# rpng/cpi

Measured on AMD Instinct MI355X. Metric: preintegration windows/sec (50-sample windows), higher is better.
Workload: dtype f64; 1 GPU; v1_mean: 10000 windows x 50 samples per GPU per step, CPI model 1, mean-only (BASELINE.json configs[1]); pool_batches=12, library_build=3afb5072f8491ca2, launch_mode=1923 timed steps replayed as ONE HIP graph (one kernel node per step), parallelism=1 GPU

## Files before the change

### cpi_amd/_lib.py

```python
import ctypes as C
import os

_HERE = os.path.dirname(os.path.abspath(__file__))
LIB_PATH = os.environ.get("CPI_AMD_LIB") or os.path.join(_HERE, "libcpi_amd.so")

CPI_OK, CPI_ERR_INVALID, CPI_ERR_HIP, CPI_ERR_NO_DEVICE, CPI_ERR_RCCL = 0, 1, 2, 3, 4
ABI_VERSION = 3
OUT_FIELDS = [("DT", 1), ("alpha", 3), ("beta", 3), ("q", 4), ("J_q", 9), ("J_a", 9), ("J_b", 9),
              ("H_a", 9), ("H_b", 9), ("O_a", 9), ("O_b", 9), ("P", 225), ("P_sym", 120)]
TRI_DOUBLES = 120


class CpiParams(C.Structure):
    _fields_ = [("sigma_w", C.c_double), ("sigma_wb", C.c_double), ("sigma_a", C.c_double),
                ("sigma_ab", C.c_double), ("grav", C.c_double * 3), ("model", C.c_int32),
                ("imu_avg", C.c_int32), ("state_transition_jacobians", C.c_int32),
                ("lanes_per_window", C.c_int32)]


class CpiOutputs(C.Structure):
    _fields_ = [(name, C.c_void_p) for name, _ in OUT_FIELDS]


class CpiLmParams(C.Structure):
# ... 27 lines not shown
    from . import build as _build
    hipcc_missing = None if (os.path.exists(_build.HIPCC) or shutil.which(_build.HIPCC)) else "no %s on this machine" % _build.HIPCC
    if LIB_PATH == _build.LIB and not hipcc_missing:
        if _build.stale():
            _build.build()
        elif _embedded_build_id(LIB_PATH) != _build.source_id():
            _build.build(force=True)
    if not os.path.exists(LIB_PATH):
        raise ImportError("cpi_amd: %s is missing and could not be built (%r); no CPU fallback exists" % (LIB_PATH, hipcc_missing))
    lib = C.CDLL(LIB_PATH)
    vp, i32, i64, dp = C.c_void_p, C.c_int32, C.c_int64, C.c_void_p
    lib.cpi_abi_version.restype = C.c_int
    if lib.cpi_abi_version() != ABI_VERSION:
        raise ImportError("cpi_amd: %s has ABI version %d, this binding expects %d (stale build?)" % (LIB_PATH, lib.cpi_abi_version(), ABI_VERSION))
    missing = [n for n in ("cpi_preintegrate_stream", "cpi_assemble_tiles", "cpi_tile_windows", "cpi_outputs_bind_slab", "cpi_preintegrate_tiled_batch_host",
                          "cpi_preintegrate_stream_host", "cpi_sqrt_information_packed_batch", "cpi_factor_eval_whitened_tri_batch",
                          "cpi_factor_hessian_tri_batch", "cpi_group_gather_chunk", "cpi_shard_chunk_bounds")
               if not hasattr(lib, n)]
    if missing:
        raise ImportError("cpi_amd: %s lacks %s (an older build: run python -m cpi_amd.build --force)" % (LIB_PATH, ", ".join(missing)))
    lib.cpi_build_id.restype = C.c_char_p
    if LIB_PATH == _build.LIB:
        have, want = (lib.cpi_build_id() or b"").decode(), _build.source_id()
        if have != want:
            msg = "cpi_amd: %s was built from other sources than this tree holds (build id %s, sources %s)%s" % (
                LIB_PATH, have, want, "; hipcc is not available here (%r)" % (hipcc_missing,) if hipcc_missing else "")
            if os.environ.get("CPI_AMD_ALLOW_STALE") != "1":
                raise ImportError(msg + " -- run python -m cpi_amd.build --force, or set CPI_AMD_ALLOW_STALE=1 to load it anyway")
            import warnings
            warnings.warn(msg + " (CPI_AMD_ALLOW_STALE=1: loaded anyway)")
    lib.cpi_group_create.argtypes = [C.c_int, C.POINTER(C.c_int), C.POINTER(vp)]
    lib.cpi_group_destroy.argtypes = [vp]
    lib.cpi_group_destroy.restype = None
    lib.cpi_group_size.argtypes = [vp]
    lib.cpi_group_ctx.argtypes = [vp, C.c_int]
    lib.cpi_group_ctx.restype = vp
    lib.cpi_group_last_error.argtypes = [vp]
    lib.cpi_group_last_error.restype = C.c_char_p
    lib.cpi_shard_bounds.argtypes = [i64, C.c_int, C.c_int, C.POINTER(i64), C.POINTER(i64)]
    lib.cpi_shard_bounds.restype = None
    lib.cpi_group_gather.argtypes = [vp, C.c_int, i64, C.POINTER(CpiOutputs), C.POINTER(CpiOutputs)]
    lib.cpi_group_gather_chunk.argtypes = [vp, C.c_int, i64, C.c_int, C.c_int, C.POINTER(CpiOutputs), C.POINTER(CpiOutputs)]
    lib.cpi_shard_chunk_bounds.argtypes = [i64, C.c_int, C.c_int, C.c_int, C.c_int, C.POINTER(i64), C.POINTER(i64)]
    lib.cpi_shard_chunk_bounds.restype = None
    lib.cpi_group_synchronize.argtypes = [vp]
    lib.cpi_ctx_create.argtypes = [C.c_int, vp, C.POINTER(vp)]
    lib.cpi_ctx_destroy.argtypes = [vp]
    lib.cpi_ctx_destroy.restype = None
    lib.cpi_last_error.argtypes = [vp]
    lib.cpi_last_error.restype = C.c_char_p
    lib.cpi_ctx_synchronize.argtypes = [vp]
    lib.cpi_ctx_set_stream.argtypes = [vp, vp]
    lib.cpi_ctx_set_capture_overlap.argtypes = [vp, i32]
    lib.cpi_preintegrate_batch.argtypes = [vp, C.POINTER(CpiParams), i64, i32, dp, vp, vp, dp, dp, C.POINTER(CpiOutputs)]
    lib.cpi_preintegrate_tiled_batch.argtypes = [vp, C.POINTER(CpiParams), i64, i32, dp, vp, dp, dp, C.POINTER(CpiOutputs)]
    lib.cpi_tile_knots.argtypes = [vp, i64, i32, dp, dp]
    lib.cpi_stream_workspace_bytes.argtypes = [i64]
    lib.cpi_stream_workspace_bytes.restype = C.c_size_t
    lib.cpi_stream_counts.argtypes = [vp, i64]
    lib.cpi_stream_counts.restype = C.c_void_p
    lib.cpi_preintegrate_stream.argtypes = [vp, C.POINTER(CpiParams), i64, dp, i64, dp, i32, dp, dp, vp, C.POINTER(CpiOutputs)]
    lib.cpi_preintegrate_stream.restype = C.c_int
    lib.cpi_preintegrate_stream_host.argtypes = [vp, C.POINTER(CpiParams), i64, dp, i64, dp, i32, dp, dp, C.POINTER(CpiOutputs), vp]
    lib.cpi_streams_workspace_bytes.argtypes = [i64, i64]
    lib.cpi_streams_workspace_bytes.restype = C.c_size_t
    lib.cpi_preintegrate_streams.argtypes = [vp, C.POINTER(CpiParams), i64, i64, dp, vp, i64, dp, vp, i32, dp, dp, vp, C.POINTER(CpiOutputs)]
    lib.cpi_preintegrate_streams_host.argtypes = [vp, C.POINTER(CpiParams), i64, i64, dp, vp, i64, dp, vp, i32, dp, dp, C.POINTER(CpiOutputs), vp]
    lib.cpi_tile_windows.argtypes = [vp, i64, i32, dp, vp, vp, dp]
    lib.cpi_assemble_tiles.argtypes = [vp, i64, dp, i64, dp, i32, dp, vp]
    lib.cpi_preintegrate_tiled_batch_host.argtypes = [vp, C.POINTER(CpiParams), i64, i32, dp, vp, dp, dp, C.POINTER(CpiOutputs)]
    lib.cpi_outputs_slab_doubles.argtypes = [C.POINTER(CpiOutputs), i64]
    lib.cpi_outputs_slab_doubles.restype = C.c_size_t
    lib.cpi_outputs_bind_slab.argtypes = [C.POINTER(CpiOutputs), i64, dp, C.POINTER(CpiOutputs)]
    lib.cpi_group_last_gather_messages.argtypes = [vp]
    if hasattr(lib, "cpi_test_group_create_shared"):
        lib.cpi_test_group_create_shared.argtypes = [C.c_int, C.c_int, C.POINTER(vp)]
        lib.cpi_test_group_create_shared.restype = C.c_int
        lib.cpi_test_quat_ops.argtypes = [vp, i32, i64, dp, dp]
        lib.cpi_test_quat_ops.restype = C.c_int
    lib.cpi_factor_eval_batch.argtypes = [vp, i32, C.POINTER(C.c_double), i64, C.POINTER(CpiOutputs), dp, dp, dp, i64, vp, vp, dp, dp, dp]
    lib.cpi_factor_eval_packed_batch.argtypes = [vp, i32, C.POINTER(C.c_double), i64, C.POINTER(CpiOutputs), dp, dp, dp, i64, vp, vp, dp]
    lib.cpi_sqrt_information_batch.argtypes = [vp, i64, dp, dp]
    lib.cpi_sqrt_information_packed_batch.argtypes = [vp, i64, dp, dp]
    lib.cpi_factor_eval_whitened_tri_batch.argtypes = [vp, i32, C.POINTER(C.c_double), i64, C.POINTER(CpiOutputs), dp, dp, dp, i64, vp, vp, dp, dp, dp, dp]
    lib.cpi_factor_hessian_tri_batch.argtypes = [vp, i32, C.POINTER(C.c_double), i64, C.POINTER(CpiOutputs), dp, dp, dp, i64, vp, vp, dp, dp]
    lib.cpi_factor_eval_whitened_batch.argtypes = [vp, i32, C.POINTER(C.c_double), i64, C.POINTER(CpiOutputs), dp, dp, dp, i64, vp, vp, dp, dp, dp, dp]
    lib.cpi_factor_hessian_batch.argtypes = [vp, i32, C.POINTER(C.c_double), i64, C.POINTER(CpiOutputs), dp, dp, dp, i64, vp, vp, dp, dp]
    lib.cpi_predict_batch.argtypes = [vp, i32, C.POINTER(C.c_double), i64, C.POINTER(CpiOutputs), dp, i64, vp, dp]
    lib.cpi_preintegrate_batch_host.argtypes = [vp, C.POINTER(CpiParams), i64, i32, dp, vp, vp, i64, dp, dp, C.POINTER(CpiOutputs)]
    lib.cpi_carry_doubles.argtypes = [i32]
    lib.cpi_carry_doubles.restype = C.c_size_t
    lib.cpi_preintegrate_resume.argtypes = [vp, C.POINTER(CpiParams), i64, i32, dp, vp, vp, dp, dp, dp, dp, C.POINTER(CpiOutputs)]
    lib.cpi_preintegrate_resume_host.argtypes = [vp, C.POINTER(CpiParams), i64, i32, dp, vp, vp, i64, dp, dp, dp, dp, C.POINTER(CpiOutputs)]
    lib.cpi_preintegrate_running.argtypes = [vp, C.POINTER(CpiParams), i64, i32, dp, vp, vp, dp, dp, C.POINTER(CpiOutputs)]
    lib.cpi_preintegrate_running_host.argtypes = [vp, C.POINTER(CpiParams), i64, i32, dp, vp, vp, i64, dp, dp, C.POINTER(CpiOutputs)]
    lib.cpi_preintegrate_running_resume.argtypes = lib.cpi_preintegrate_resume.argtypes
    lib.cpi_preintegrate_running_resume_host.argtypes = lib.cpi_preintegrate_resume_host.argtypes
    lib.cpi_preintegrate_running_resume.restype = lib.cpi_preintegrate_running_resume_host.restype = C.c_int
    lib.cpi_query_batch.argtypes = [vp, C.POINTER(CpiParams), i64, i32, dp, vp, vp, dp, dp, C.POINTER(CpiOutputs), i64, vp, dp, C.POINTER(CpiOutputs)]
    lib.cpi_query_batch_host.argtypes = [vp, C.POINTER(CpiParams), i64, i32, dp, vp, vp, i64, dp, dp, i64, vp, dp, C.POINTER(CpiOutputs)]
    lib.cpi_query_batch.restype = lib.cpi_query_batch_host.restype = C.c_int
    lib.cpi_query_cov_batch.argtypes = lib.cpi_query_batch.argtypes
    lib.cpi_query_cov_batch_host.argtypes = lib.cpi_query_batch_host.argtypes
    lib.cpi_query_cov_batch.restype = lib.cpi_query_cov_batch_host.restype = C.c_int
    lib.cpi_query_stj_batch.argtypes = lib.cpi_query_cov_batch.argtypes
    lib.cpi_query_stj_batch_host.argtypes = lib.cpi_query_cov_batch_host.argtypes
# ... 77 lines not shown
```

### cpi_amd/csrc/cpi_abi.hip

```cpp
#include <hip/hip_runtime.h>
#include <rccl/rccl.h>
#include <dlfcn.h>
#include <stdlib.h>
#include <stdint.h>
#include <stdio.h>
#include <string.h>
#include <algorithm>
#include <cmath>
#include <mutex>
#include <string>
#include <vector>

#include "../../include/cpi_amd.h"
#ifdef CPI_TEST_HOOKS
#include "../../include/cpi_amd_test.h"
#endif
#include "cpi_args.hpp"
#include "cpi_capture_overlap.hpp"

using namespace cpi;

constexpr int kOutFields = 13;
static_assert(sizeof(cpi_outputs) == kOutFields * sizeof(double *), "cpi_outputs is a plain table of kOutFields pointers");
static const int OUT_N[kOutFields] = { 1, 3, 3, 4, 9, 9, 9, 9, 9, 9, 9, 225, CPI_TRI_DOUBLES };
static double **out_field(cpi_outputs *o, int k) {
    double **f[kOutFields] = { &o->DT, &o->alpha, &o->beta, &o->q, &o->J_q, &o->J_a, &o->J_b, &o->H_a, &o->H_b, &o->O_a, &o->O_b, &o->P, &o->P_sym };
    return f[k];
}
static double *out_field_c(const cpi_outputs *o, int k) { cpi_outputs t = *o; return *out_field(&t, k); }

struct HostPipe;
static void host_pipe_destroy(HostPipe *);
struct cpi_ctx {
    int device;
    hipStream_t stream;
    std::string err;
    hipStream_t side = nullptr;
    hipEvent_t ev_fork = nullptr, ev_join = nullptr;
    unsigned big_lds_set = 0;
    struct HostPipe *pipe = nullptr;
    int overlap_depth = 1;
    bool overlap_allowed = true;
    overlap::Window<hipGraphNode_t> window;
    std::vector<hipGraphNode_t> ov_found, ov_preds;
};
static thread_local std::string g_create_err;

static int fail(cpi_ctx *ctx, int code, const std::string &msg) {
    if (ctx) ctx->err = msg; else g_create_err = msg;
    return code;
}
struct DeviceGuard {
    int prev = -1;
    bool changed = false;
    hipError_t enter(int dev) {
        hipError_t e = hipGetDevice(&prev);
        if (e != hipSuccess) return e;
        if (prev == dev) return hipSuccess;
        e = hipSetDevice(dev);
        changed = (e == hipSuccess);
        return e;
    }
    ~DeviceGuard() { if (changed) (void)hipSetDevice(prev); }
};
#define CPI_HIP(ctx, call)                                                                      \
    do {                                                                                        \
        hipError_t e_ = (call);                                                                 \
        if (e_ != hipSuccess)                                                                   \
            return fail(ctx, CPI_ERR_HIP, std::string(#call) + ": " + hipGetErrorString(e_));   \
    } while (0)

extern "C" int cpi_abi_version(void) { return CPI_ABI_VERSION; }
#ifndef CPI_BUILD_ID
#define CPI_BUILD_ID "unknown"
#endif
static const char kBuildIdTagged[] = "cpi-build-id:" CPI_BUILD_ID;
extern "C" const char *cpi_build_id(void) { return kBuildIdTagged + 13; }

extern "C" int cpi_ctx_create(int device, void *stream, cpi_ctx **out) {
    if (!out) return fail(nullptr, CPI_ERR_INVALID, "cpi_ctx_create: out is NULL");
    *out = nullptr;
    int ndev = 0;
    hipError_t e = hipGetDeviceCount(&ndev);
    if (e != hipSuccess || ndev <= 0)
        return fail(nullptr, CPI_ERR_NO_DEVICE, "cpi_ctx_create: no HIP device available (this library has no CPU fallback)");
    if (device < 0) {
        e = hipGetDevice(&device);
        if (e != hipSuccess) return fail(nullptr, CPI_ERR_HIP, std::string("hipGetDevice: ") + hipGetErrorString(e));
    }
    if (device >= ndev) return fail(nullptr, CPI_ERR_INVALID, "cpi_ctx_create: device index out of range");
    cpi_ctx *c = new cpi_ctx();
    c->device = device;
    c->stream = (hipStream_t)stream;
    const overlap::Policy pol = overlap::policy_from_environment();
    c->overlap_allowed = pol.allowed;
    c->overlap_depth = pol.depth;
    *out = c;
    return CPI_OK;
}
extern "C" void cpi_ctx_destroy(cpi_ctx *ctx) {
    if (!ctx) return;
    if (ctx->side || ctx->pipe) {
        int prev = -1;
        (void)hipGetDevice(&prev);
        (void)hipSetDevice(ctx->device);
        if (ctx->side) {
            (void)hipStreamDestroy(ctx->side);
            (void)hipEventDestroy(ctx->ev_fork);
            (void)hipEventDestroy(ctx->ev_join);
        }
        if (ctx->pipe) host_pipe_destroy(ctx->pipe);
        if (prev >= 0) (void)hipSetDevice(prev);
    }
    delete ctx;
}
extern "C" int cpi_ctx_set_stream(cpi_ctx *ctx, void *stream) {
    if (!ctx) return fail(nullptr, CPI_ERR_INVALID, "ctx is NULL");
    if (ctx->stream != (hipStream_t)stream) ctx->window.close();
    ctx->stream = (hipStream_t)stream;
    return CPI_OK;
}
extern "C" int cpi_ctx_set_capture_overlap(cpi_ctx *ctx, int32_t depth) {
    if (!ctx) return fail(nullptr, CPI_ERR_INVALID, "ctx is NULL");
    ctx->overlap_depth = ctx->overlap_allowed ? overlap::clamp_depth(depth) : 1;
    ctx->window.close();
    return CPI_OK;
}
extern "C" const char *cpi_last_error(const cpi_ctx *ctx) { return ctx ? ctx->err.c_str() : g_create_err.c_str(); }
extern "C" int cpi_ctx_synchronize(cpi_ctx *ctx) {
    if (!ctx) return fail(nullptr, CPI_ERR_INVALID, "ctx is NULL");
    DeviceGuard guard_;
    CPI_HIP(ctx, guard_.enter(ctx->device));
    CPI_HIP(ctx, hipStreamSynchronize(ctx->stream));
    return CPI_OK;
}

static bool grid_ok(long long nb) { return nb > 0 && nb <= 0x7fffffffLL; }

#ifdef CPI_EXPERIMENTS
namespace expsw {
static launch::MeanDmaCfg mean_dma() {
    static launch::MeanDmaCfg c = [] {
        launch::MeanDmaCfg d = {0, 0, 0};
        const char *e = getenv("CPI_AMD_MEAN_DMA");
        if (e && strcmp(e, "off") != 0) { int k = 0, s = 0, al = 1; if (sscanf(e, "%d,%d,%d", &k, &s, &al) >= 2) d = {k, s, al}; }
        return d;
    }();
    return c;
}
static int env_int(const char *name, int dflt) { const char *e = getenv(name); return e ? atoi(e) : dflt; }
static int mean_blk() { static int v = [] { const char *e = getenv("CPI_AMD_MEAN_BLK"); return e ? (strcmp(e, "off") == 0 ? -1 : atoi(e)) : 0; }(); return v; }
static bool mean_line() { static int v = env_int("CPI_AMD_MEAN_LINE", 0); return v != 0; }
static int blk_mode() { static int v = env_int("CPI_AMD_BLK_MODE", 0); return v; }
static int probe_lds() { static int v = env_int("CPI_AMD_PROBE_LDS", 0); return v; }
static bool no_overlap() { static int v = env_int("CPI_AMD_NO_OVERLAP", 0); return v != 0; }
static bool no_fused_cut() { static int v = env_int("CPI_AMD_NO_FUSED_CUT", 0); return v != 0; }
static int factor_lanes() { static int v = env_int("CPI_AMD_FACTOR_LANES", 0); return (v == 16 || v == 8 || v == 4) ? v : 0; }
static int cost_lanes() { static int v = env_int("CPI_AMD_COST_LANES", 0); return (v == 16 || v == 8 || v == 4) ? v : 0; }
static int packed_lpf() { static int v = env_int("CPI_AMD_PACKED_LPF", 0); return (v == 2 || v == 3 || v == 4 || v == 6 || v == 8) ? v : 0; }
}
#endif

static int pick_lanes(const cpi_params *prm, int64_t W, int N, bool jac) {
    if (prm->model == CPI_MODEL_V2 && jac) return 1;
    const double t_int = (prm->model == CPI_MODEL_V2) ? 1.2 : 0.55, t_lvl = (prm->model == CPI_MODEL_V2) ? 1.3 : 0.3;
    int L = prm->lanes_per_window;
    if (L <= 0) {
        double best = 1e300;
        L = 1;
        const int *choices = nullptr;
        const int nc = launch::mean_lane_choices(&choices);
        for (int i = 0; i < nc; i++) {
            const int c = choices[i];
            if (c > 1 && 2 * c > N) break;
            const int64_t waves = (W + (64 / c) - 1) / (64 / c);
            if (c > 1 && waves > 1024) break;
            int levels = 0;
            while ((1 << levels) < c) levels++;
// ... 77 lines not shown
                         const double *lin, const double *q_k_lin) {
    if (!knots || !lin) return refuse(ctx, who, "knots/lin is NULL");
    CPI_TRY(check_qk(ctx, who, prm, q_k_lin));
    CPI_TRY(check_grid(ctx, who, "W", W, " (32-bit grid)"));
    CPI_TRY(check_N(ctx, who, N));
    return check_lanes(ctx, prm);
}
static int check_carry_overlap(cpi_ctx *ctx, const char *who, const cpi_params *prm, int64_t W, const double *carry_in, const double *carry_out) {
    const int64_t n = W * (int64_t)carry::doubles(prm->model);
    return (carry_in && carry_in < carry_out + n && carry_out < carry_in + n) ? refuse(ctx, who, "carry_in and carry_out overlap") : CPI_OK;
}
static int carry_header(const cpi_params *prm) {
    const bool stj = prm->model == CPI_MODEL_V2 && prm->state_transition_jacobians != 0;
    return 1 | (prm->imu_avg != 0 ? 8 : 0) | (stj ? 16 : 0) | (32 * prm->model);
}

static int side_fork(cpi_ctx *ctx) {
    if (!ctx->side) {
        CPI_HIP(ctx, hipStreamCreateWithFlags(&ctx->side, hipStreamNonBlocking));
        CPI_HIP(ctx, hipEventCreateWithFlags(&ctx->ev_fork, hipEventDisableTiming));
        CPI_HIP(ctx, hipEventCreateWithFlags(&ctx->ev_join, hipEventDisableTiming));
    }
    CPI_HIP(ctx, hipEventRecord(ctx->ev_fork, ctx->stream));
    CPI_HIP(ctx, hipStreamWaitEvent(ctx->side, ctx->ev_fork, 0));
    return CPI_OK;
}
static int side_join(cpi_ctx *ctx) {
    CPI_HIP(ctx, hipEventRecord(ctx->ev_join, ctx->side));
    CPI_HIP(ctx, hipStreamWaitEvent(ctx->stream, ctx->ev_join, 0));
    return CPI_OK;
}

struct StreamCut {
    long long K;
    const double *update;
    long long *first;
    int *count;
    double *tstart, *tend;
    const RunArgs *runs;
};
static int cut_launch(cpi_ctx *ctx, const StreamCut &sc, const double *stream, int64_t U, int32_t N) {
    if (sc.runs) launch::cut_runs(sc.K, stream, (long long)U, sc.update, *sc.runs, sc.first, sc.count, sc.tstart, sc.tend, ctx->stream);
    else launch::cut_windows(sc.K, stream, (long long)U, sc.update, (int)N, sc.first, sc.count, sc.tstart, sc.tend, ctx->stream);
    CPI_HIP(ctx, hipGetLastError());
    return CPI_OK;
}
static void overlap_give_up(cpi_ctx *ctx, bool restore) {
    (void)hipGetLastError();
    if (restore) {
        (void)hipStreamUpdateCaptureDependencies(ctx->stream, ctx->ov_found.empty() ? nullptr : ctx->ov_found.data(), ctx->ov_found.size(),
                                                 hipStreamAddCaptureDependencies);
        (void)hipGetLastError();
    }
    ctx->window.close();
}
static bool capture_overlap_begin(cpi_ctx *ctx, const overlap::Footprint &fp) {
    if (ctx->overlap_depth <= 1 || !ctx->stream) return false;
    hipStreamCaptureStatus status = hipStreamCaptureStatusNone;
    unsigned long long id = 0;
    const hipGraphNode_t *deps = nullptr;
    size_t ndeps = 0;
    if (hipStreamGetCaptureInfo_v2(ctx->stream, &status, &id, nullptr, &deps, &ndeps) != hipSuccess) { overlap_give_up(ctx, false); return false; }
    if (status != hipStreamCaptureStatusActive || (ndeps && !deps)) { ctx->window.close(); return false; }
    if (!overlap::capture_registry().sole(id, ctx)) { ctx->window.close(); return false; }
    ctx->ov_found.assign(deps, deps + ndeps);
    if (!ctx->window.continues(id, ctx->ov_found.data(), ndeps)) ctx->window.open_at(id, ctx->overlap_depth, ctx->ov_found.data(), ndeps);
    ctx->window.plan(fp, ctx->ov_preds);
    if (overlap::same_set(ctx->ov_preds, ctx->ov_found.data(), ndeps)) return true;
    if (hipStreamUpdateCaptureDependencies(ctx->stream, ctx->ov_preds.empty() ? nullptr : ctx->ov_preds.data(), ctx->ov_preds.size(),
                                           hipStreamSetCaptureDependencies) != hipSuccess) {
        overlap_give_up(ctx, true);
        return false;
    }
    return true;
}
static void capture_overlap_end(cpi_ctx *ctx, const overlap::Footprint &fp) {
    hipStreamCaptureStatus status = hipStreamCaptureStatusNone;
    unsigned long long id = 0;
    const hipGraphNode_t *deps = nullptr;
    size_t ndeps = 0;
    if (hipStreamGetCaptureInfo_v2(ctx->stream, &status, &id, nullptr, &deps, &ndeps) != hipSuccess ||
        status != hipStreamCaptureStatusActive || ndeps != 1 || !deps) { overlap_give_up(ctx, true); return; }
    const hipGraphNode_t node = deps[0];
    for (hipGraphNode_t p : ctx->ov_preds) if (p == node) { overlap_give_up(ctx, true); return; }
    ctx->window.commit(node, fp);
    const std::vector<hipGraphNode_t> &fr = ctx->window.frontier();
    if (fr.size() == 1) return;
    if (hipStreamUpdateCaptureDependencies(ctx->stream, const_cast<hipGraphNode_t *>(fr.data()), fr.size(), hipStreamSetCaptureDependencies) != hipSuccess)
        overlap_give_up(ctx, true);
}

static int preintegrate_impl(cpi_ctx *ctx, const char *who, const cpi_params *prm, int64_t W, int32_t N, const double *knots,
                             const int64_t *first, const int32_t *count, const StreamCut *sc, const double *lin,
                             const double *q_k_lin, const cpi_outputs *out) {
    if (!ctx) return fail(nullptr, CPI_ERR_INVALID, "ctx is NULL");
    if (!prm || !out) return refuse(ctx, who, "prm/out is NULL");
    if (!model_is_cpi(prm) && prm->model != CPI_MODEL_FORSTER) return refuse(ctx, who, "model must be 1, 2 or 3 (CPI_MODEL_FORSTER)");
    if (W < 0 || N < 0) return refuse(ctx, who, "negative size");
    if (W == 0) return CPI_OK;
    CPI_TRY(check_windows(ctx, who, prm, W, N, knots, lin, q_k_lin));

    const Request rq = request_of(out);
    const bool forster = prm->model == CPI_MODEL_FORSTER;
    const bool avg = prm->imu_avg != 0;
    const bool v2 = prm->model == CPI_MODEL_V2;
    const bool stj = v2 && prm->state_transition_jacobians != 0;
    const bool run_cov = !forster && (rq.cov || (stj && rq.jac));
    const bool mean_jac = !forster && rq.jac && !stj;
    const bool run_mean = !forster && (mean_jac || (rq.mean && !run_cov));
    bool fused_cut = sc && rq.any() && run_mean && !mean_jac && !run_cov && (sc->runs != nullptr || sc->K >= 4);
#ifdef CPI_EXPERIMENTS
    if (expsw::no_fused_cut()) fused_cut = false;
#endif

    bool overlap_ok = !sc && run_mean && !run_cov;
#ifdef CPI_EXPERIMENTS
    overlap_ok = overlap_ok && expsw::mean_blk() <= 0 && expsw::mean_dma().kc <= 0 && !expsw::mean_line();
#endif

    DeviceGuard guard_;
    CPI_HIP(ctx, guard_.enter(ctx->device));
    if (!overlap_ok) ctx->window.close();
    if (sc && !fused_cut) {
        CPI_TRY(cut_launch(ctx, *sc, knots, W, N));
        first = reinterpret_cast<const int64_t *>(sc->first); count = sc->count;
    }
    if (!rq.any()) return CPI_OK;
    PreArgs a = pre_args(prm, W, N, knots, first, count, lin, q_k_lin, out);
    if (sc) { a.K = sc->K; if (!fused_cut) { a.tstart = sc->tstart; a.tend = sc->tend; } }
    if (forster) {
        launch::forster(a, ctx->stream);
        CPI_HIP(ctx, hipGetLastError());
        return CPI_OK;
    }

    bool forked = run_cov && run_mean && mean_jac;
#ifdef CPI_EXPERIMENTS
    forked = forked && !expsw::no_overlap();
#endif
    if (forked) CPI_TRY(side_fork(ctx));
    const hipStream_t mean_stream = forked ? ctx->side : ctx->stream;
    if (run_cov) {
        PreArgs c = a;
        c.write_means = rq.mean ? 1 : 0;
        c.write_jac = (stj && rq.jac) ? 1 : 0;
        launch::cov(prm->model, avg, c, ctx->stream);
    }
    if (run_mean) {
        PreArgs m = a;
        m.write_means = (rq.mean && !run_cov) ? 1 : 0;
        m.write_jac = mean_jac ? 1 : 0;
        if (fused_cut) { m.update = sc->update; m.count_out = sc->count; m.first = nullptr; m.count = nullptr; }
        const int LL = pick_lanes(prm, W, N, mean_jac);
        long long done = 0;
#ifdef CPI_EXPERIMENTS
        const int bl = expsw::mean_blk();
        m.dbg = expsw::blk_mode();
        if (!sc && !mean_jac && !first && bl > 0 && (size_t)(64 / bl) * (size_t)(N + 1) * 56 <= 65536 && N >= 1) {
            if (launch::mean_blk(prm->model, bl, avg, m, ctx->stream)) done = W;
        }
        const launch::MeanDmaCfg dc = expsw::mean_dma();
        if (!sc && !done && !mean_jac && LL == 1 && !first && !count && dc.kc > 0 && N >= 2 * dc.kc)
            done = launch::mean_dma(prm->model, dc, avg, m, ctx->stream);
        if (!sc && !done && !mean_jac && LL == 1 && !first && !count && expsw::mean_line()) done = launch::mean_line(prm->model, avg, m, ctx->stream);
        if (done && done < W) m = shift_windows(m, done);
#endif
        if (done < W) {
            if (fused_cut && sc->runs) launch::mean_runs(prm->model, avg, LL, m, *sc->runs, mean_stream);
            else if (overlap_ok && ctx->overlap_depth > 1 && !overlap::launch_is_latency_bound((W + (64 / LL) - 1) / (64 / LL))) {
                ctx->window.close();
                launch::mean(prm->model, mean_jac, avg, LL, m, mean_stream);
            } else if (overlap_ok && ctx->overlap_depth > 1) {
                const void *outs[kOutFields];
                for (int k = 0; k < kOutFields; k++) outs[k] = out_field_c(out, k);
                const overlap::Footprint fp = overlap::make_footprint(W, N, knots, first, count, lin, q_k_lin, outs, OUT_N, kOutFields);
                const bool in_window = capture_overlap_begin(ctx, fp);
                launch::mean(prm->model, mean_jac, avg, LL, m, mean_stream);
                const hipError_t launched = hipGetLastError();
                if (in_window) capture_overlap_end(ctx, fp);
                CPI_HIP(ctx, launched);
            } else launch::mean(prm->model, mean_jac, avg, LL, m, mean_stream);
        }
    }
    if (forked) CPI_TRY(side_join(ctx));
    CPI_HIP(ctx, hipGetLastError());
    return CPI_OK;
}
extern "C" int cpi_preintegrate_batch(cpi_ctx *ctx, const cpi_params *prm, int64_t W, int32_t N,
                                      const double *knots, const int64_t *first, const int32_t *count,
                                      const double *lin, const double *q_k_lin, const cpi_outputs *out) {
    return preintegrate_impl(ctx, "cpi_preintegrate_batch", prm, W, N, knots, first, count, nullptr, lin, q_k_lin, out);
}

extern "C" size_t cpi_carry_doubles(int32_t model) { return (model == CPI_MODEL_V1 || model == CPI_MODEL_V2) ? (size_t)carry::doubles(model) : 0; }
extern "C" int cpi_preintegrate_resume(cpi_ctx *ctx, const cpi_params *prm, int64_t W, int32_t N,
                                       const double *knots, const int64_t *first, const int32_t *count,
                                       const double *lin, const double *q_k_lin, const double *carry_in, double *carry_out,
                                       const cpi_outputs *out) {
    static const char who[] = "cpi_preintegrate_resume";
    if (!ctx) return fail(nullptr, CPI_ERR_INVALID, "ctx is NULL");
    if (!prm || !out) return refuse(ctx, who, "prm/out is NULL");
    if (!model_is_cpi(prm)) return refuse_forster(ctx, who, NOT_RESUMABLE);
    if (!carry_out) return refuse(ctx, who, "carry_out is NULL");
    if (W < 0 || N < 0) return refuse(ctx, who, "negative size");
    CPI_TRY(check_carry_overlap(ctx, who, prm, W, carry_in, carry_out));
    if (W == 0) return CPI_OK;
    CPI_TRY(check_windows(ctx, who, prm, W, N, knots, lin, q_k_lin));

    const Request rq = request_of(out);
    const bool avg = prm->imu_avg != 0;
    const bool stj = prm->model == CPI_MODEL_V2 && prm->state_transition_jacobians != 0;
    const bool run_cov = rq.cov || (stj && rq.jac);
    const bool mean_jac = rq.jac && !stj;
    const bool run_mean = mean_jac || !run_cov;
    CarryArgs c;
    c.in = carry_in;
    c.out = carry_out;
    c.need = carry_header(prm) | (run_cov ? carry::TAG_P : 0) | (mean_jac ? carry::TAG_J : 0);
    c.tag_out = c.need;

    DeviceGuard guard_;
    CPI_HIP(ctx, guard_.enter(ctx->device));
    const PreArgs a = pre_args(prm, W, N, knots, first, count, lin, q_k_lin, out);
    const bool forked = run_cov && run_mean;
    if (forked) CPI_TRY(side_fork(ctx));
    if (run_cov) {
        PreArgs p = a;
        p.write_means = rq.mean ? 1 : 0;
        p.write_jac = (stj && rq.jac) ? 1 : 0;
        CarryArgs cc = c;
        cc.own_means = 1;
        launch::cov_carry(prm->model, avg, p, cc, ctx->stream);
// ... 2616 lines not shown
```

### cpi_amd/csrc/cpi_capture_overlap.hpp

```cpp
#pragma once
#include <stddef.h>
#include <stdint.h>
#include <stdlib.h>
#include <mutex>
#include <vector>

namespace cpi {
namespace overlap {

constexpr int kMaxDepth = 4;
constexpr int kDefaultDepth = 2;
inline int clamp_depth(long long d) { return d < 1 ? 1 : (d > kMaxDepth ? kMaxDepth : (int)d); }

struct Policy {
    bool allowed;
    int depth;
};
inline Policy policy_from(const char *hw_queues, const char *depth) {
    Policy p;
    p.allowed = !(hw_queues && *hw_queues && atoll(hw_queues) < 4);
    p.depth = p.allowed ? clamp_depth(depth && *depth ? atoll(depth) : kDefaultDepth) : 1;
    return p;
}
inline Policy policy_from_environment() { return policy_from(getenv("GPU_MAX_HW_QUEUES"), getenv("CPI_AMD_CAPTURE_OVERLAP")); }
// ... 77 lines not shown
class Window {
public:
    bool is_open() const { return open_; }
    void close() { open_ = false; }
    long long calls() const { return n_; }
    const std::vector<Node> &base() const { return base_; }
    const std::vector<Node> &frontier() const { return frontier_; }

    bool continues(unsigned long long capture_id, const Node *deps, size_t ndeps) const {
        return open_ && capture_id == id_ && same_set(frontier_, deps, ndeps);
    }
    void open_at(unsigned long long capture_id, int depth, const Node *deps, size_t ndeps) {
        open_ = true; id_ = capture_id; depth_ = clamp_depth(depth); n_ = 0;
        base_.assign(deps, deps + ndeps);
        frontier_ = base_;
    }
    void plan(const Footprint &fp, std::vector<Node> &preds) {
        preds.clear();
        const long long i = n_, D = depth_;
        uint32_t anc = 0;
        for (long long d = 1; d <= 2 * D - 1 && d <= i; d++) {
            const long long j = i - d;
            if ((anc >> d) & 1u) continue;
            if (d < D && !conflict(fp_[j % kRing], fp)) continue;
            preds.push_back(node_[j % kRing]);
            anc |= (1u << d) | (anc_[j % kRing] << d) | (~0u << (d + D));
        }
        if (preds.empty()) preds = base_;
        pending_anc_ = anc;
    }
    void commit(Node node, const Footprint &fp) {
        node_[n_ % kRing] = node; fp_[n_ % kRing] = fp; anc_[n_ % kRing] = pending_anc_;
        n_++;
        frontier_.clear();
        for (long long j = n_ - 1; j >= 0 && j >= n_ - depth_; j--) {
            bool covered = false;
            for (long long l = j + 1; l < n_ && !covered; l++) covered = (anc_[l % kRing] >> (l - j)) & 1u;
            if (!covered) frontier_.push_back(node_[j % kRing]);
        }
    }

private:
    static constexpr int kRing = 2 * kMaxDepth;
    bool open_ = false;
    unsigned long long id_ = 0;
    int depth_ = 1;
    long long n_ = 0;
    std::vector<Node> base_, frontier_;
    Node node_[kRing] = {};
    Footprint fp_[kRing];
    uint32_t anc_[kRing] = {}, pending_anc_ = 0;
};

}
}
```

### cpi_amd/engine.py

```python
import ctypes as C
from ctypes import byref

import numpy as np
import torch

from . import _lib
from ._lib import OUT_FIELDS, CpiError, CpiLmParams, CpiOutputs, CpiParams

DEFAULT_SIGMAS = (0.005, 4e-6, 0.01, 2e-4)
DEFAULT_GRAV = (0.0, 0.0, 9.8)
MEAN_FIELDS = ("DT", "alpha", "beta", "q")
JAC_FIELDS = ("J_q", "J_a", "J_b", "H_a", "H_b", "O_a", "O_b")


def _group_of(name):
    if name in MEAN_FIELDS:
        return "mean"
    return "cov" if name == "P" else ("cov_sym" if name == "P_sym" else "jac")


def _ptr(t):
    return None if t is None else C.c_void_p(t.data_ptr())


# ... 34 lines not shown
class _nullctx:
    def __enter__(self):
        return None

    def __exit__(self, *a):
        return False


class Engine:

    def __init__(self, device=None, stream=None):
        self.lib = _lib.load()
        self._follow = stream is None
        if device is None:
            device = torch.cuda.current_device() if torch.cuda.is_available() else 0
        self.device = torch.device("cuda", device) if isinstance(device, int) else torch.device(device)
        ctx = C.c_void_p()
        if stream is None and torch.cuda.is_available():
            stream = torch.cuda.current_stream(self.device)
        sptr = C.c_void_p(stream.cuda_stream) if stream is not None else None
        rc = self.lib.cpi_ctx_create(self.device.index or 0, sptr, C.byref(ctx))
        if rc != 0:
            raise CpiError(rc, (self.lib.cpi_last_error(None) or b"").decode())
        self.ctx = ctx
        self.stream = stream

    def close(self):
        if getattr(self, "ctx", None):
            self.lib.cpi_ctx_destroy(self.ctx)
            self.ctx = None

    def __del__(self):
        try:
            self.close()
        except Exception:
            pass

    def _check(self, rc):
        if rc != 0:
            raise CpiError(rc, (self.lib.cpi_last_error(self.ctx) or b"").decode())

    def _sync_stream(self):
        if self._follow:
            cur = torch.cuda.current_stream(self.device)
            if cur.cuda_stream != self.stream.cuda_stream:
                self._check(self.lib.cpi_ctx_set_stream(self.ctx, C.c_void_p(cur.cuda_stream)))
                self.stream = cur

    def synchronize(self):
        self._check(self.lib.cpi_ctx_synchronize(self.ctx))

    def set_capture_overlap(self, depth):
        self._check(self.lib.cpi_ctx_set_capture_overlap(self.ctx, int(depth)))

    @staticmethod
    def make_params(model=1, imu_avg=False, state_transition_jacobians=True, sigmas=DEFAULT_SIGMAS,
                    grav=DEFAULT_GRAV, lanes_per_window=0):
        p = CpiParams()
        p.sigma_w, p.sigma_wb, p.sigma_a, p.sigma_ab = sigmas
        p.grav[:] = grav
        p.model, p.imu_avg = int(model), int(bool(imu_avg))
        p.state_transition_jacobians = int(bool(state_transition_jacobians))
        p.lanes_per_window = int(lanes_per_window)
        return p

    def alloc_outputs(self, W, want=("mean", "jac", "cov"), model=1, packed=False):
        names = []
        for name, n in OUT_FIELDS:
            grp = _group_of(name)
            if grp not in want:
                continue
            if model != 2 and name in ("O_a", "O_b"):
                continue
            names.append((name, n))
        out = {}
        if packed:
            from .dist import alloc_packed
            flat, out = alloc_packed(names, W, self.device)
            out["_flat"], out["_fields"] = flat, names
            return out
        for name, n in names:
            shape = (W,) if n == 1 else (W, n)
            out[name] = torch.empty(shape, dtype=torch.float64, device=self.device)
        return out

    @staticmethod
    def _outputs_struct(out):
        o = CpiOutputs()
        for name, _ in OUT_FIELDS:
            t = out.get(name)
            setattr(o, name, t.data_ptr() if t is not None else None)
        return o

    @staticmethod
    def _window_shape(knots, lin, first=None, count=None, N=None, others=(), cuda=True):
        if first is None:
            W, n1, _ = knots.shape
            N = n1 - 1
        else:
            W = first.shape[0]
            assert N is not None, "ragged layout needs N = max intervals per window"
        for t in (knots, lin, first, count) + tuple(others):
            assert t is None or (t.is_cuda == cuda and t.is_contiguous()), "inputs must be contiguous %s tensors" % ("CUDA" if cuda else "CPU")
        assert knots.dtype == torch.float64 and lin.dtype == torch.float64 and (count is None or count.dtype == torch.int32)
        return W, N

# ... 1558 lines not shown
```

### include/cpi_amd.h

```cpp
#ifndef CPI_AMD_H
#define CPI_AMD_H

#include <stddef.h>
#include <stdint.h>

#ifdef __cplusplus
extern "C" {
#endif

#define CPI_ABI_VERSION 3

enum { CPI_OK = 0, CPI_ERR_INVALID = 1, CPI_ERR_HIP = 2, CPI_ERR_NO_DEVICE = 3, CPI_ERR_RCCL = 4 };
enum {
    CPI_MODEL_V1 = 1, CPI_MODEL_V2 = 2,
    CPI_MODEL_FORSTER = 3
};

typedef struct cpi_ctx cpi_ctx;

typedef struct {
    double sigma_w, sigma_wb, sigma_a, sigma_ab;
    double grav[3];
    int32_t model;
    int32_t imu_avg;
    int32_t state_transition_jacobians;
    int32_t lanes_per_window;
} cpi_params;

typedef struct {
    double *DT;
    double *alpha;
    double *beta;
    double *q;
    double *J_q;
    double *J_a;
    double *J_b;
    double *H_a;
    double *H_b;
    double *O_a;
    double *O_b;
    double *P;
    double *P_sym;
} cpi_outputs;

#define CPI_TRI_DOUBLES 120
#define CPI_TRI_INDEX(i, j) ((i) + (j) * ((j) + 1) / 2)

int cpi_ctx_create(int device, void *stream, cpi_ctx **out);
void cpi_ctx_destroy(cpi_ctx *ctx);
int cpi_ctx_set_stream(cpi_ctx *ctx, void *stream);
int cpi_ctx_set_capture_overlap(cpi_ctx *ctx, int32_t depth);
const char *cpi_last_error(const cpi_ctx *ctx);
int cpi_abi_version(void);
const char *cpi_build_id(void);
int cpi_ctx_synchronize(cpi_ctx *ctx);

int cpi_preintegrate_batch(cpi_ctx *ctx, const cpi_params *prm, int64_t W, int32_t N,
                           const double *knots, const int64_t *first, const int32_t *count,
                           const double *lin, const double *q_k_lin, const cpi_outputs *out);

size_t cpi_carry_doubles(int32_t model);
int cpi_preintegrate_resume(cpi_ctx *ctx, const cpi_params *prm, int64_t W, int32_t N,
                            const double *knots, const int64_t *first, const int32_t *count,
                            const double *lin, const double *q_k_lin, const double *carry_in, double *carry_out,
                            const cpi_outputs *out);

int cpi_preintegrate_running(cpi_ctx *ctx, const cpi_params *prm, int64_t W, int32_t N,
                             const double *knots, const int64_t *first, const int32_t *count,
                             const double *lin, const double *q_k_lin, const cpi_outputs *rows);

int cpi_preintegrate_running_resume(cpi_ctx *ctx, const cpi_params *prm, int64_t W, int32_t N,
                                    const double *knots, const int64_t *first, const int32_t *count,
                                    const double *lin, const double *q_k_lin,
                                    const double *carry_in, double *carry_out, const cpi_outputs *rows);

int cpi_query_batch(cpi_ctx *ctx, const cpi_params *prm, int64_t W, int32_t N,
                    const double *knots, const int64_t *first, const int32_t *count,
                    const double *lin, const double *q_k_lin, const cpi_outputs *rows,
                    int64_t Q, const int32_t *qwin, const double *qtime, const cpi_outputs *out);

int cpi_query_cov_batch(cpi_ctx *ctx, const cpi_params *prm, int64_t W, int32_t N,
                        const double *knots, const int64_t *first, const int32_t *count,
                        const double *lin, const double *q_k_lin, const cpi_outputs *rows,
                        int64_t Q, const int32_t *qwin, const double *qtime, const cpi_outputs *out);

int cpi_running_stj_batch(cpi_ctx *ctx, const cpi_params *prm, int64_t W, int32_t N,
                          const double *knots, const int64_t *first, const int32_t *count,
                          const double *lin, const double *q_k_lin, const cpi_outputs *rows);

int cpi_query_stj_batch(cpi_ctx *ctx, const cpi_params *prm, int64_t W, int32_t N,
                        const double *knots, const int64_t *first, const int32_t *count,
                        const double *lin, const double *q_k_lin, const cpi_outputs *rows,
                        int64_t Q, const int32_t *qwin, const double *qtime, const cpi_outputs *out);

int cpi_running_resume_stj_batch(cpi_ctx *ctx, const cpi_params *prm, int64_t W, int32_t N,
                                 const double *knots, const int64_t *first, const int32_t *count,
                                 const double *lin, const double *q_k_lin,
                                 const double *carry_in, double *carry_out, const cpi_outputs *rows);

int cpi_query_open_batch(cpi_ctx *ctx, const cpi_params *prm, int64_t W, int32_t N,
                         const double *knots, const int64_t *first, const int32_t *count,
                         const double *lin, const double *q_k_lin, const cpi_outputs *rows,
                         int64_t Q, const int32_t *qwin, const double *qtime, const cpi_outputs *out,
                         const cpi_outputs *base, int32_t base_N);
// ... 267 lines not shown
```

Before: 1.013 billion windows/s.

## Add strand-based capture overlap scheduler and make it the default

Adds a 'strands' mode for building graph dependencies during stream capture. Each captured mean kernel is assigned to one of up to four parallel chains, picked by read/write range conflicts or, when nothing conflicts, by least-recent use. Before this, a lookback window limited overlap to a fixed depth. Independent kernel nodes in the replayed graph can now run concurrently with fewer serialising edges, which should help small, latency-bound launches. In exchange it adds conflict-tracking overhead at capture time, and a mistake in the range tracking could let kernels that touch the same memory run at the same time.

```diff
diff --git a/cpi_amd/_lib.py b/cpi_amd/_lib.py
--- a/cpi_amd/_lib.py
+++ b/cpi_amd/_lib.py
@@ -103,6 +103,7 @@
     lib.cpi_ctx_synchronize.argtypes = [vp]
     lib.cpi_ctx_set_stream.argtypes = [vp, vp]
     lib.cpi_ctx_set_capture_overlap.argtypes = [vp, i32]
+    lib.cpi_ctx_set_capture_strands.argtypes = [vp, i32]
     lib.cpi_preintegrate_batch.argtypes = [vp, C.POINTER(CpiParams), i64, i32, dp, vp, vp, dp, dp, C.POINTER(CpiOutputs)]
     lib.cpi_preintegrate_tiled_batch.argtypes = [vp, C.POINTER(CpiParams), i64, i32, dp, vp, dp, dp, C.POINTER(CpiOutputs)]
     lib.cpi_tile_knots.argtypes = [vp, i64, i32, dp, dp]
diff --git a/cpi_amd/csrc/cpi_abi.hip b/cpi_amd/csrc/cpi_abi.hip
--- a/cpi_amd/csrc/cpi_abi.hip
+++ b/cpi_amd/csrc/cpi_abi.hip
@@ -39,9 +39,12 @@
     hipEvent_t ev_fork = nullptr, ev_join = nullptr;
     unsigned big_lds_set = 0;
     struct HostPipe *pipe = nullptr;
-    int overlap_depth = 1;
+    overlap::Shape overlap_shape = overlap::kShapeLookback;
+    int overlap_n = 1;
     bool overlap_allowed = true;
     overlap::Window<hipGraphNode_t> window;
+    overlap::Strands<hipGraphNode_t> strands;
+    void close_window() { window.close(); strands.close(); }
     std::vector<hipGraphNode_t> ov_found, ov_preds;
 };
 static thread_local std::string g_create_err;
@@ -92,9 +95,10 @@
     cpi_ctx *c = new cpi_ctx();
     c->device = device;
     c->stream = (hipStream_t)stream;
-    const overlap::Policy pol = overlap::policy_from_environment();
+    const overlap::CapturePolicy pol = overlap::capture_policy_from_environment();
     c->overlap_allowed = pol.allowed;
-    c->overlap_depth = pol.depth;
+    c->overlap_shape = pol.shape;
+    c->overlap_n = pol.n;
     *out = c;
     return CPI_OK;
 }
@@ -116,14 +120,22 @@
 }
 extern "C" int cpi_ctx_set_stream(cpi_ctx *ctx, void *stream) {
     if (!ctx) return fail(nullptr, CPI_ERR_INVALID, "ctx is NULL");
-    if (ctx->stream != (hipStream_t)stream) ctx->window.close();
+    if (ctx->stream != (hipStream_t)stream) ctx->close_window();
     ctx->stream = (hipStream_t)stream;
     return CPI_OK;
 }
 extern "C" int cpi_ctx_set_capture_overlap(cpi_ctx *ctx, int32_t depth) {
     if (!ctx) return fail(nullptr, CPI_ERR_INVALID, "ctx is NULL");
-    ctx->overlap_depth = ctx->overlap_allowed ? overlap::clamp_depth(depth) : 1;
-    ctx->window.close();
+    ctx->overlap_shape = overlap::kShapeLookback;
+    ctx->overlap_n = ctx->overlap_allowed ? overlap::clamp_depth(depth) : 1;
+    ctx->close_window();
+    return CPI_OK;
+}
+extern "C" int cpi_ctx_set_capture_strands(cpi_ctx *ctx, int32_t n) {
+    if (!ctx) return fail(nullptr, CPI_ERR_INVALID, "ctx is NULL");
+    ctx->overlap_shape = overlap::kShapeStrands;
+    ctx->overlap_n = ctx->overlap_allowed ? overlap::clamp_strands(n) : 1;
+    ctx->close_window();
     return CPI_OK;
 }
 extern "C" const char *cpi_last_error(const cpi_ctx *ctx) { return ctx ? ctx->err.c_str() : g_create_err.c_str(); }
@@ -307,20 +319,21 @@
                                                  hipStreamAddCaptureDependencies);
         (void)hipGetLastError();
     }
-    ctx->window.close();
-}
-static bool capture_overlap_begin(cpi_ctx *ctx, const overlap::Footprint &fp) {
-    if (ctx->overlap_depth <= 1 || !ctx->stream) return false;
+    ctx->close_window();
+}
+template <class Win>
+static bool capture_overlap_begin(cpi_ctx *ctx, Win &win, const overlap::Footprint &fp) {
+    if (ctx->overlap_n <= 1 || !ctx->stream) return false;
     hipStreamCaptureStatus status = hipStreamCaptureStatusNone;
     unsigned long long id = 0;
     const hipGraphNode_t *deps = nullptr;
     size_t ndeps = 0;
     if (hipStreamGetCaptureInfo_v2(ctx->stream, &status, &id, nullptr, &deps, &ndeps) != hipSuccess) { overlap_give_up(ctx, false); return false; }
-    if (status != hipStreamCaptureStatusActive || (ndeps && !deps)) { ctx->window.close(); return false; }
-    if (!overlap::capture_registry().sole(id, ctx)) { ctx->window.close(); return false; }
+    if (status != hipStreamCaptureStatusActive || (ndeps && !deps)) { win.close(); return false; }
+    if (!overlap::capture_registry().sole(id, ctx)) { win.close(); return false; }
     ctx->ov_found.assign(deps, deps + ndeps);
-    if (!ctx->window.continues(id, ctx->ov_found.data(), ndeps)) ctx->window.open_at(id, ctx->overlap_depth, ctx->ov_found.data(), ndeps);
-    ctx->window.plan(fp, ctx->ov_preds);
+    if (!win.continues(id, ctx->ov_found.data(), ndeps)) win.open_at(id, ctx->overlap_n, ctx->ov_found.data(), ndeps);
+    win.plan(fp, ctx->ov_preds);
     if (overlap::same_set(ctx->ov_preds, ctx->ov_found.data(), ndeps)) return true;
     if (hipStreamUpdateCaptureDependencies(ctx->stream, ctx->ov_preds.empty() ? nullptr : ctx->ov_preds.data(), ctx->ov_preds.size(),
                                            hipStreamSetCaptureDependencies) != hipSuccess) {
@@ -329,7 +342,8 @@
     }
     return true;
 }
-static void capture_overlap_end(cpi_ctx *ctx, const overlap::Footprint &fp) {
+template <class Win>
+static void capture_overlap_end(cpi_ctx *ctx, Win &win, const overlap::Footprint &fp) {
     hipStreamCaptureStatus status = hipStreamCaptureStatusNone;
     unsigned long long id = 0;
     const hipGraphNode_t *deps = nullptr;
@@ -338,9 +352,9 @@
         status != hipStreamCaptureStatusActive || ndeps != 1 || !deps) { overlap_give_up(ctx, true); return; }
     const hipGraphNode_t node = deps[0];
     for (hipGraphNode_t p : ctx->ov_preds) if (p == node) { overlap_give_up(ctx, true); return; }
-    ctx->window.commit(node, fp);
-    const std::vector<hipGraphNode_t> &fr = ctx->window.frontier();
-    if (fr.size() == 1) return;
+    win.commit(node, fp);
+    const std::vector<hipGraphNode_t> &fr = win.frontier();
+    if (fr.size() == 1 && fr[0] == node) return;
     if (hipStreamUpdateCaptureDependencies(ctx->stream, const_cast<hipGraphNode_t *>(fr.data()), fr.size(), hipStreamSetCaptureDependencies) != hipSuccess)
         overlap_give_up(ctx, true);
 }
@@ -375,7 +389,7 @@
 
     DeviceGuard guard_;
     CPI_HIP(ctx, guard_.enter(ctx->device));
-    if (!overlap_ok) ctx->window.close();
+    if (!overlap_ok) ctx->close_window();
     if (sc && !fused_cut) {
         CPI_TRY(cut_launch(ctx, *sc, knots, W, N));
         first = reinterpret_cast<const int64_t *>(sc->first); count = sc->count;
@@ -422,17 +436,18 @@
 #endif
         if (done < W) {
             if (fused_cut && sc->runs) launch::mean_runs(prm->model, avg, LL, m, *sc->runs, mean_stream);
-            else if (overlap_ok && ctx->overlap_depth > 1 && !overlap::launch_is_latency_bound((W + (64 / LL) - 1) / (64 / LL))) {
-                ctx->window.close();
+            else if (overlap_ok && ctx->overlap_n > 1 && !overlap::launch_is_latency_bound((W + (64 / LL) - 1) / (64 / LL))) {
+                ctx->close_window();
                 launch::mean(prm->model, mean_jac, avg, LL, m, mean_stream);
-            } else if (overlap_ok && ctx->overlap_depth > 1) {
+            } else if (overlap_ok && ctx->overlap_n > 1) {
                 const void *outs[kOutFields];
                 for (int k = 0; k < kOutFields; k++) outs[k] = out_field_c(out, k);
                 const overlap::Footprint fp = overlap::make_footprint(W, N, knots, first, count, lin, q_k_lin, outs, OUT_N, kOutFields);
-                const bool in_window = capture_overlap_begin(ctx, fp);
+                const bool strands = ctx->overlap_shape == overlap::kShapeStrands;
+                const bool in_window = strands ? capture_overlap_begin(ctx, ctx->strands, fp) : capture_overlap_begin(ctx, ctx->window, fp);
                 launch::mean(prm->model, mean_jac, avg, LL, m, mean_stream);
                 const hipError_t launched = hipGetLastError();
-                if (in_window) capture_overlap_end(ctx, fp);
+                if (in_window) { if (strands) capture_overlap_end(ctx, ctx->strands, fp); else capture_overlap_end(ctx, ctx->window, fp); }
                 CPI_HIP(ctx, launched);
             } else launch::mean(prm->model, mean_jac, avg, LL, m, mean_stream);
         }
diff --git a/cpi_amd/csrc/cpi_capture_overlap.hpp b/cpi_amd/csrc/cpi_capture_overlap.hpp
--- a/cpi_amd/csrc/cpi_capture_overlap.hpp
+++ b/cpi_amd/csrc/cpi_capture_overlap.hpp
@@ -153,5 +153,154 @@
     uint32_t anc_[kRing] = {}, pending_anc_ = 0;
 };
 
-}
-}
+constexpr int kMaxStrands = 4;
+constexpr int kReadRanges = 64, kWriteRanges = 32;
+inline int clamp_strands(long long n) { return n < 1 ? 1 : (n > kMaxStrands ? kMaxStrands : (int)n); }
+
+template <int Cap>
+class RangeSet {
+public:
+    int size() const { return n_; }
+    const Range &operator[](int i) const { return r_[i]; }
+    void clear() { n_ = 0; }
+    bool overlaps(const Range &x) const {
+        if (x.hi <= x.lo) return false;
+        int i = 0;
+        while (i < n_ && r_[i].hi <= x.lo) i++;
+        return i < n_ && r_[i].lo < x.hi;
+    }
+    bool add(const Range &x) {
+        if (x.hi <= x.lo) return true;
+        int i = 0;
+        while (i < n_ && r_[i].hi < x.lo) i++;
+        int j = i;
+        while (j < n_ && r_[j].lo <= x.hi) j++;
+        if (i == j) {
+            if (n_ == Cap) return false;
+            for (int k = n_; k > i; k--) r_[k] = r_[k - 1];
+            r_[i] = x;
+            n_++;
+            return true;
+        }
+        Range m = {x.lo < r_[i].lo ? x.lo : r_[i].lo, x.hi > r_[j - 1].hi ? x.hi : r_[j - 1].hi};
+        r_[i] = m;
+        for (int k = j; k < n_; k++) r_[i + 1 + (k - j)] = r_[k];
+        n_ -= j - i - 1;
+        return true;
+    }
+
+private:
+    int n_ = 0;
+    Range r_[Cap];
+};
+
+template <class Node, int RCap = kReadRanges, int WCap = kWriteRanges>
+class Strands {
+public:
+    bool is_open() const { return open_; }
+    void close() { open_ = false; }
+    long long calls() const { return n_; }
+    long long joins() const { return joins_; }
+    int last_strand() const { return last_; }
+    const std::vector<Node> &base() const { return base_; }
+    const std::vector<Node> &frontier() const { return frontier_; }
+
+    bool continues(unsigned long long capture_id, const Node *deps, size_t ndeps) const {
+        return open_ && capture_id == id_ && same_set(frontier_, deps, ndeps);
+    }
+    void open_at(unsigned long long capture_id, int strands, const Node *deps, size_t ndeps) {
+        open_ = true; id_ = capture_id; S_ = clamp_strands(strands); n_ = 0; joins_ = 0; last_ = -1;
+        base_.assign(deps, deps + ndeps);
+        restart();
+    }
+    void plan(const Footprint &fp, std::vector<Node> &preds) {
+        preds.clear();
+        int hit = -1, nhit = 0, nonempty = 0, lru = 0;
+        for (int s = 0; s < S_; s++) {
+            if (!st_[s].empty) nonempty++;
+            if (conflicts(st_[s], fp)) { nhit++; hit = s; }
+            if (st_[s].stamp < st_[lru].stamp) lru = s;
+        }
+        target_ = nhit == 0 ? lru : hit;
+        if (nhit >= 2 || (fp.unknown && nonempty >= 2)) target_ = -1;
+        if (target_ >= 0) {
+            pending_ = st_[target_];
+            pending_.everything = pending_.everything || fp.unknown;
+            bool fits = true;
+            if (!fp.unknown) {
+                for (int k = 0; k < fp.nr && fits; k++) fits = pending_.reads.add(fp.r[k]);
+                for (int k = 0; k < fp.nw && fits; k++) fits = pending_.writes.add(fp.w[k]);
+            }
+            if (!fits) target_ = -1;
+        }
+        if (target_ >= 0) {
+            if (!st_[target_].empty) preds.push_back(st_[target_].tail);
+        } else {
+            for (int s = 0; s < S_; s++) if (!st_[s].empty) preds.push_back(st_[s].tail);
+        }
+        if (preds.empty()) preds = base_;
+    }
+    void commit(Node node, const Footprint &) {
+        n_++;
+        last_ = target_;
+        if (target_ < 0) {
+            joins_++;
+            base_.assign(1, node);
+            restart();
+            return;
+        }
+        st_[target_] = pending_;
+        st_[target_].empty = false; st_[target_].tail = node; st_[target_].stamp = ++clock_;
+        frontier_.clear();
+        for (int s = 0; s < S_; s++) if (!st_[s].empty) frontier_.push_back(st_[s].tail);
+    }
+
+private:
+    struct Strand {
+        bool empty = true, everything = false;
+        Node tail = Node();
+        unsigned long long stamp = 0;
+        RangeSet<RCap> reads;
+        RangeSet<WCap> writes;
+    };
+    static bool conflicts(const Strand &s, const Footprint &fp) {
+        if (s.empty) return false;
+        if (s.everything || fp.unknown) return true;
+        for (int k = 0; k < fp.nw; k++) if (s.reads.overlaps(fp.w[k]) || s.writes.overlaps(fp.w[k])) return true;
+        for (int k = 0; k < fp.nr; k++) if (s.writes.overlaps(fp.r[k])) return true;
+        return false;
+    }
+    void restart() {
+        for (int s = 0; s < kMaxStrands; s++) { st_[s].empty = true; st_[s].everything = false; st_[s].stamp = 0; st_[s].reads.clear(); st_[s].writes.clear(); }
+        clock_ = 0;
+        frontier_ = base_;
+    }
+
+    bool open_ = false;
+    unsigned long long id_ = 0, clock_ = 0;
+    int S_ = 1, target_ = -1, last_ = -1;
+    long long n_ = 0, joins_ = 0;
+    std::vector<Node> base_, frontier_;
+    Strand st_[kMaxStrands], pending_;
+};
+
+enum Shape { kShapeLookback = 0, kShapeStrands = 1 };
+constexpr int kDefaultStrands = 4;
+constexpr Shape kDefaultShape = kShapeStrands;
+struct CapturePolicy {
+    bool allowed;
+    Shape shape;
+    int n;
+};
+inline CapturePolicy capture_policy_from(const char *hw_queues, const char *strands, const char *depth) {
+    if (hw_queues && *hw_queues && atoll(hw_queues) < 4) return {false, kDefaultShape, 1};
+    if (strands && *strands) return {true, kShapeStrands, clamp_strands(atoll(strands))};
+    if (depth && *depth) return {true, kShapeLookback, clamp_depth(atoll(depth))};
+    return {true, kDefaultShape, kDefaultShape == kShapeStrands ? kDefaultStrands : kDefaultDepth};
+}
+inline CapturePolicy capture_policy_from_environment() {
+    return capture_policy_from(getenv("GPU_MAX_HW_QUEUES"), getenv("CPI_AMD_CAPTURE_STRANDS"), getenv("CPI_AMD_CAPTURE_OVERLAP"));
+}
+
+}
+}
diff --git a/cpi_amd/engine.py b/cpi_amd/engine.py
--- a/cpi_amd/engine.py
+++ b/cpi_amd/engine.py
@@ -110,6 +110,9 @@
 
     def set_capture_overlap(self, depth):
         self._check(self.lib.cpi_ctx_set_capture_overlap(self.ctx, int(depth)))
+
+    def set_capture_strands(self, n):
+        self._check(self.lib.cpi_ctx_set_capture_strands(self.ctx, int(n)))
 
     @staticmethod
     def make_params(model=1, imu_avg=False, state_transition_jacobians=True, sigmas=DEFAULT_SIGMAS,
diff --git a/include/cpi_amd.h b/include/cpi_amd.h
--- a/include/cpi_amd.h
+++ b/include/cpi_amd.h
@@ -50,6 +50,7 @@
 void cpi_ctx_destroy(cpi_ctx *ctx);
 int cpi_ctx_set_stream(cpi_ctx *ctx, void *stream);
 int cpi_ctx_set_capture_overlap(cpi_ctx *ctx, int32_t depth);
+int cpi_ctx_set_capture_strands(cpi_ctx *ctx, int32_t n);
 const char *cpi_last_error(const cpi_ctx *ctx);
 int cpi_abi_version(void);
 const char *cpi_build_id(void);
```

Measured after the change: 1.116 billion windows/s (median of 6 runs). 10.1% higher.
